# hammershock/3dgs-avatar-release

Measured on AMD Instinct MI355X. Metric: render fps (fwd+bwd) @200k Gaussians 1024x1024 SH3, higher is better.
Workload: dtype f32; 1 GPU; config3: 200k Gaussians, 1024x1024, SH deg 3, forward+backward; shs+scales+rotations inputs, L1 loss (L1 fused into the rasterizer: l1_target); tile_rect=1, l1=fused, long_lists=0, gaussians=200000, width=1024, height=1024, sh_degree=3, frames_per_rank=1857, total_frames=1857, ranks=1, backend=none, parallelism=frames sharded x1

## Files before the change

### 3dgs-avatar-release_amd/csrc/render_bwd.hip

```cpp
#include "common.h"
#include "blend.h"

__device__ __forceinline__ float ring_ror1(float v) {
    return __builtin_bit_cast(float, __builtin_amdgcn_update_dpp(0, __builtin_bit_cast(int, v), 0x121, 0xF, 0xF, true));
}
#define RING 16
#define RING_STRIDE 48

typedef float bwd_f4 __attribute__((ext_vector_type(4)));
template <bool SECOND>
__device__ __forceinline__ void split_accumulate(float (&x)[9], float (&y)[9], unsigned long long mask, float Gd, float dx,
                                                 float dy, float tdx, float tdy, float wgt, float gx, float gy,
                                                 float gz, unsigned long long m1, uint32_t lds_addr, bwd_f4& q0, bwd_f4& q1,
                                                 bwd_f4& q2, float& rot0, float& rot1) {
    unsigned long long save;
    asm volatile(
        "s_mov_b64 %[sv], exec\n\t"
        "s_mov_b64 exec, %[m]\n\t"
        "v_fmac_f32 %[x0], %[Gd], %[dx]\n\t"
        "v_fmac_f32 %[x1], %[Gd], %[dy]\n\t"
        "v_fmac_f32 %[x2], %[tdx], %[dx]\n\t"
        "v_fmac_f32 %[x3], %[tdx], %[dy]\n\t"
        "v_fmac_f32 %[x4], %[tdy], %[dy]\n\t"
        "v_add_f32 %[x5], %[x5], %[Gd]\n\t"
        "v_fmac_f32 %[x6], %[w], %[gx]\n\t"
        "v_fmac_f32 %[x7], %[w], %[gy]\n\t"
        "v_fmac_f32 %[x8], %[w], %[gz]\n\t"
        "s_mov_b64 exec, %[sv]"
        : [x0] "+v"(x[0]), [x1] "+v"(x[1]), [x2] "+v"(x[2]), [x3] "+v"(x[3]), [x4] "+v"(x[4]), [x5] "+v"(x[5]), [x6] "+v"(x[6]),
          [x7] "+v"(x[7]), [x8] "+v"(x[8]), [sv] "=&s"(save)
        : [m] "s"(mask), [Gd] "v"(Gd), [dx] "v"(dx), [dy] "v"(dy), [tdx] "v"(tdx), [tdy] "v"(tdy), [w] "v"(wgt), [gx] "v"(gx),
          [gy] "v"(gy), [gz] "v"(gz)
        : "scc");
#define GS_ACC_Y                                     \
        "s_andn2_b64 exec, %[sv], %[m]\n\t"          \
        "v_fmac_f32 %[y0], %[Gd], %[dx]\n\t"         \
        "v_fmac_f32 %[y1], %[Gd], %[dy]\n\t"         \
        "v_fmac_f32 %[y2], %[tdx], %[dx]\n\t"        \
        "v_fmac_f32 %[y3], %[tdx], %[dy]\n\t"        \
        "v_fmac_f32 %[y4], %[tdy], %[dy]\n\t"        \
        "v_add_f32 %[y5], %[y5], %[Gd]\n\t"          \
        "v_fmac_f32 %[y6], %[w], %[gx]\n\t"          \
        "v_fmac_f32 %[y7], %[w], %[gy]\n\t"          \
        "v_fmac_f32 %[y8], %[w], %[gz]\n\t"          \
        "s_mov_b64 exec, %[sv]\n\t"                  \
        "v_mov_b32_dpp %[r0], %[r0] row_ror:1 row_mask:0xf bank_mask:0xf bound_ctrl:1\n\t" \
        "v_mov_b32_dpp %[r1], %[r1] row_ror:1 row_mask:0xf bank_mask:0xf bound_ctrl:1\n\t" \
        "s_waitcnt lgkmcnt(0)"
#define GS_ACC_Y_OUT [y0] "+v"(y[0]), [y1] "+v"(y[1]), [y2] "+v"(y[2]), [y3] "+v"(y[3]), [y4] "+v"(y[4]), [y5] "+v"(y[5]), \
                     [y6] "+v"(y[6]), [y7] "+v"(y[7]), [y8] "+v"(y[8]), [q0] "+v"(q0), [q1] "+v"(q1), [r0] "+v"(rot0), [r1] "+v"(rot1), \
                     [sv] "=&s"(save)
#define GS_ACC_Y_IN [m] "s"(mask), [m1] "s"(m1), [a] "v"(lds_addr), [Gd] "v"(Gd), [dx] "v"(dx), [dy] "v"(dy), [tdx] "v"(tdx), \
                    [tdy] "v"(tdy), [w] "v"(wgt), [gx] "v"(gx), [gy] "v"(gy), [gz] "v"(gz)
    if constexpr (SECOND) {
        asm volatile(
            "s_mov_b64 %[sv], exec\n\t"
            "s_andn2_b64 exec, %[m1], %[m]\n\t"
            "ds_read_b128 %[q0], %[a]\n\t"
            "ds_read_b128 %[q1], %[a] offset:16\n\t"
            "ds_read_b128 %[q2], %[a] offset:32\n\t" GS_ACC_Y
            : GS_ACC_Y_OUT, [q2] "+v"(q2)
            : GS_ACC_Y_IN
            : "memory", "scc");
    } else {
        asm volatile(
            "s_mov_b64 %[sv], exec\n\t"
            "s_andn2_b64 exec, %[m1], %[m]\n\t"
            "ds_read_b128 %[q0], %[a]\n\t"
            "ds_read_b128 %[q1], %[a] offset:16\n\t"
            "ds_read_b32 %[q2], %[a] offset:32\n\t" GS_ACC_Y
            : GS_ACC_Y_OUT, [q2] "+v"(q2.x)
            : GS_ACC_Y_IN
            : "memory", "scc");
    }
#undef GS_ACC_Y
#undef GS_ACC_Y_OUT
#undef GS_ACC_Y_IN
}

struct EntryQ {
    bwd_f4 q0, q1, q2;
};
#define ENT_SLOTS 2

template <bool SECOND>
__device__ __forceinline__ void switch_entry(EntryQ& e, uint32_t lds_addr, unsigned long long m0, unsigned long long m1) {
    unsigned long long save;
    if constexpr (SECOND) {
        asm volatile(
            "s_mov_b64 %[sv], exec\n\t"
            "s_andn2_b64 exec, %[m1], %[m0]\n\t"
            "ds_read_b128 %[q0], %[a]\n\t"
            "ds_read_b128 %[q1], %[a] offset:16\n\t"
            "ds_read_b128 %[q2], %[a] offset:32\n\t"
            "s_mov_b64 exec, %[sv]\n\t"
            "s_waitcnt lgkmcnt(0)"
            : [q0] "+v"(e.q0), [q1] "+v"(e.q1), [q2] "+v"(e.q2), [sv] "=&s"(save)
            : [a] "v"(lds_addr), [m0] "s"(m0), [m1] "s"(m1)
            : "memory", "scc");
    } else {
        float b = e.q2.x;
        asm volatile(
            "s_mov_b64 %[sv], exec\n\t"
            "s_andn2_b64 exec, %[m1], %[m0]\n\t"
            "ds_read_b128 %[q0], %[a]\n\t"
            "ds_read_b128 %[q1], %[a] offset:16\n\t"
            "ds_read_b32 %[b], %[a] offset:32\n\t"
            "s_mov_b64 exec, %[sv]\n\t"
            "s_waitcnt lgkmcnt(0)"
            : [q0] "+v"(e.q0), [q1] "+v"(e.q1), [b] "+v"(b), [sv] "=&s"(save)
            : [a] "v"(lds_addr), [m0] "s"(m0), [m1] "s"(m1)
            : "memory", "scc");
        e.q2.x = b;
    }
}

#ifndef BWD_MIN_WAVES
#define BWD_MIN_WAVES 1
#endif
template <int MODE>
__global__ __launch_bounds__(64, BWD_MIN_WAVES) void render_bwd_kernel(const float4* __restrict__ rec,
                                                        const uint2* __restrict__ ranges,
                                                        const uint32_t* __restrict__ order, int W, int H, int gx,
                                                        int ntiles, int xmap,
                                                        const uint32_t* __restrict__ qlist,
                                                        const uint32_t* __restrict__ ncon_c,
                                                        const uint32_t* __restrict__ qcount,
                                                        const float* __restrict__ out_color,
                                                        const float* __restrict__ dL_dpix,
                                                        const float* __restrict__ dL_dopa,
                                                        const float* __restrict__ final_T, const float* __restrict__ bg,
                                                        float4* __restrict__ qrows, uint32_t* __restrict__ q8,
                                                        const float4* __restrict__ ckpt,
                                                        const uint32_t* __restrict__ ck_start, const int chunks,
                                                        const int blocks_per_chunk, const SecondImage second,
                                                        const L1Grad l1, const float l1_inv_n) {
    constexpr bool OPA = MODE == 1, SECOND = MODE == 2, SONES = MODE == 3;
    if constexpr (SECOND) { if (*second.all_ones != 0u) return; }
    if constexpr (SONES) { if (*second.all_ones == 0u) return; }
    constexpr int NP2 = SECOND ? 5 : 3;
    __shared__ float2 pix[NP2][4 * RING_STRIDE];
    __shared__ bwd_f4 ent[ENT_SLOTS][RING][3];
    int slot, q;
    const int chunk = chunks > 1 ? (int)blockIdx.x / blocks_per_chunk : 0;
    render_block_map((int)blockIdx.x - chunk * blocks_per_chunk, xmap, &slot, &q);
    if (slot >= ntiles) return;
    const int tile = (int)(order[slot] & 0x7FFFFFFFu);
    const int tx = tile % gx, ty = tile / gx;
    const int lane = threadIdx.x;
    const int j = lane & (RING - 1), ring = lane / RING;
    const int QX0 = tx * TILE + 8 * (q & 1), QY0 = ty * TILE + 8 * (q >> 1);
    const int px = QX0 + (lane & 7), py = QY0 + (lane >> 3);
    const uint2 range = ranges[tile];
    const int n = (int)(range.y - range.x);
    const int m_all = (int)qcount[tile * 4 + q];
    const uint32_t ks = chunk > 0 ? ck_start[(size_t)(tile * 4 + q) * (size_t)chunks + chunk] : 0u;
    if (ks >= (uint32_t)m_all) return;
    const int k0 = (int)ks;
    const uint32_t ke = chunk + 1 < chunks ? ck_start[(size_t)(tile * 4 + q) * (size_t)chunks + chunk + 1] : 0xFFFFFFFFu;
    const int m = (int)min(ke, (uint32_t)m_all) - k0;
    const uint32_t qbase = 4u * range.x + (uint32_t)q * (uint32_t)n + (uint32_t)k0;
    const float4 zero4 = make_float4(0.f, 0.f, 0.f, 0.f);
    float gtot0, T0 = 1.0f;
    {
        float4 c0 = zero4, c1 = make_float4((float)px, (float)py, __uint_as_float((uint32_t)j), 0.f);
        float3 h = make_float3(0.f, 0.f, 0.f);
        if (px < W && py < H) {
            const size_t HW = (size_t)H * W;
            const size_t pid = (size_t)py * W + px;
            float g0 = 0.f, g1 = 0.f, g2 = 0.f;
            if (dL_dpix) { g0 = dL_dpix[pid]; g1 = dL_dpix[HW + pid]; g2 = dL_dpix[2 * HW + pid]; }
            const float o0 = out_color[pid], o1 = out_color[HW + pid], o2 = out_color[2 * HW + pid];
            if (l1.target) {
                const float sc = (l1.grad ? l1.grad[0] : 1.0f) * l1_inv_n;
                const float d0 = o0 - l1.target[pid], d1 = o1 - l1.target[HW + pid], d2 = o2 - l1.target[2 * HW + pid];
                g0 += d0 > 0.f ? sc : (d0 < 0.f ? -sc : 0.f);
                g1 += d1 > 0.f ? sc : (d1 < 0.f ? -sc : 0.f);
                g2 += d2 > 0.f ? sc : (d2 < 0.f ? -sc : 0.f);
            }
            c0 = make_float4(g0, g1, g2, o0 * g0 + o1 * g1 + o2 * g2);
            const uint32_t nc = ncon_c[pid];
            c1.z = __uint_as_float((nc > (uint32_t)k0 ? nc - (uint32_t)k0 : 0u) + (uint32_t)j);
            if (OPA) {
                const float Tf = final_T[pid];
                c0.w -= dL_dopa[pid] * (Tf * (1.0f - bg[0]));
            }
            if (SECOND || SONES) {
                h = make_float3(second.dL_dpix[pid], second.dL_dpix[HW + pid], second.dL_dpix[2 * HW + pid]);
                if (SECOND) c0.w += second.out_color[pid] * h.x + second.out_color[HW + pid] * h.y + second.out_color[2 * HW + pid] * h.z;
                else c0.w -= (1.0f - second.out_color[pid]) * h.x + (1.0f - second.out_color[HW + pid]) * h.y + (1.0f - second.out_color[2 * HW + pid]) * h.z;
            }
            if (chunk > 0) {
                const size_t ci = ((size_t)(tile * 4 + q) * (size_t)(chunks - 1) + (size_t)(chunk - 1)) * 64 + lane;
                const float4 ck = ckpt[ci];
                T0 = ck.x;
                c0.w -= ck.y * g0 + ck.z * g1 + ck.w * g2;
                if (SECOND) {
                    const float4 ck2 = second.ckpt[ci];
                    c0.w -= ck2.y * h.x + ck2.z * h.y + ck2.w * h.z;
                }
            }
        }
        const int slot = ring * RING_STRIDE + j;
        pix[0][slot] = pix[0][slot + RING] = make_float2(c0.x, c0.y);
        pix[1][slot] = pix[1][slot + RING] = make_float2(c0.z, c1.x);
        pix[2][slot] = pix[2][slot + RING] = make_float2(c1.y, c1.z);
        if (SECOND) {
            pix[3][slot] = pix[3][slot + RING] = make_float2(h.x, h.y);
            pix[4][slot] = pix[4][slot + RING] = make_float2(h.z, 0.f);
        }
        gtot0 = c0.w;
    }

    float3 q2 = make_float3(0.f, 0.f, 0.f);
    auto stage = [&](const float4 p0, const float4 p1, const float4 p2, const int chunk, uint32_t& row) {
        const uint32_t off = __float_as_uint(p2.y), rmin = __float_as_uint(p2.z), rsz = __float_as_uint(p2.w);
        const uint32_t minx = rmin & 0xFFFFu, miny = rmin >> 16, w = rsz & 0xFFFFu;
        row = gradient_row(off, w, (uint32_t)tx - minx, (uint32_t)ty - miny, (uint32_t)q);
        if (ring == 0) {
            bwd_f4* e = ent[chunk & (ENT_SLOTS - 1)][j];
            e[0] = bwd_f4{p0.x, p0.y, (-0.5f * LOG2E_F) * p0.z, -LOG2E_F * p0.w};
            e[1] = bwd_f4{(-0.5f * LOG2E_F) * p1.x, p1.y, p1.z, p1.w};
            e[2] = bwd_f4{p2.x, q2.x, q2.y, q2.z};
        }
    };
    auto gather = [&](int k, float4& p0, float4& p1, float4& p2) {
        if (k < m) {
            const uint32_t id = qlist[qbase + k];
            p0 = rec[(size_t)id * 3];
            p1 = rec[(size_t)id * 3 + 1];
            p2 = rec[(size_t)id * 3 + 2];
            if (SECOND) q2 = make_float3(second.colors[(size_t)id * 3], second.colors[(size_t)id * 3 + 1], second.colors[(size_t)id * 3 + 2]);
        }
    };

    float4 p0 = zero4, p1 = zero4, p2 = zero4;
    EntryQ cur;
    cur.q0 = cur.q1 = cur.q2 = bwd_f4{0.f, 0.f, 0.f, 0.f};
    uint32_t row_staged = 0;
    gather(j, p0, p1, p2);
    stage(p0, p1, p2, 0, row_staged);
    gather(RING + j, p0, p1, p2);
    __syncthreads();
    const uint32_t ent_addr0 = (uint32_t)(uintptr_t)&ent[0][j][0], ent_addr1 = (uint32_t)(uintptr_t)&ent[1][j][0];

    float accA[9], accB[9];
#pragma unroll
    for (int c9 = 0; c9 < 9; c9++) accA[c9] = accB[c9] = 0.f;
    uint32_t rowA = 0, rowB = 0;
    uint32_t pidx = (uint32_t)(ring * RING_STRIDE + ((RING - j) & (RING - 1)));
    float2 pc[NP2];
#pragma unroll
    for (int c6 = 0; c6 < NP2; c6++) pc[c6] = pix[c6][pidx];
    float T = __shfl(T0, ring * RING + ((RING - j) & (RING - 1)), 64);
    float Rem = __shfl(gtot0, ring * RING + ((RING - j) & (RING - 1)), 64);

    auto write_row = [&](size_t row, const float* a) {
        qrows[row * 2] = make_float4(a[0], a[1], a[2], a[3]);
        qrows[row * 2 + 1] = make_float4(a[4], a[5], a[6], a[7]);
        q8[row] = __float_as_uint(a[8]);
    };

    const int total = m + RING - 1;
    auto fold_rings = [&](float (&a)[9]) {
#pragma unroll
        for (int c9 = 0; c9 < 9; c9++) {
            a[c9] += __shfl_xor(a[c9], 16, 64);
            a[c9] += __shfl_xor(a[c9], 32, 64);
        }
    };
    auto run_round = [&](const int s0, float (&X)[9], uint32_t& rowX, float (&Y)[9]) {
        if (s0 >= 2 * RING) {
            fold_rings(X);
            if (ring == 0) write_row(rowX, X);
        }
        rowX = row_staged;
        const uint32_t ea = (s0 & RING) ? ent_addr1 : ent_addr0;
        switch_entry<SECOND>(cur, ea, 0ull, 0x0001000100010001ull);
        stage(p0, p1, p2, s0 / RING + 1, row_staged);
        gather(s0 + 2 * RING + j, p0, p1, p2);
        if (s0 > 0) pidx -= (uint32_t)RING;
#pragma unroll
        for (int c9 = 0; c9 < 9; c9++) X[c9] = 0.f;
        const int tend = min(RING, total - s0);
        unsigned long long mx = 0x0001000100010001ull;
        auto step = [&](const int t) {
            const uint32_t s = (uint32_t)(s0 + t);
            const float3 g = make_float3(pc[0].x, pc[0].y, pc[1].x);
            const float pxf = pc[1].y, pyf = pc[2].x;
            const uint32_t lim = __float_as_uint(pc[2].y);
            const float h0 = SECOND ? pc[3].x : 0.f, h1 = SECOND ? pc[3].y : 0.f, h2 = SECOND ? pc[NP2 - 1].x : 0.f;
            pidx += 1u;
#pragma unroll
            for (int c6 = 0; c6 < NP2; c6++) pc[c6] = pix[c6][pidx];
            const float dx = cur.q0.x - pxf, dy = cur.q0.y - pyf;
            const float power2 = __builtin_fmaf(cur.q0.z * dx, dx, __builtin_fmaf(cur.q0.w, dx, cur.q1.x * dy) * dy);
            const float G = __builtin_amdgcn_exp2f(power2);
            const float al = fminf(0.99f, cur.q1.y * G);
            const bool valid = (power2 <= 0.0f) && (s < lim) && (al >= (1.0f / 255.0f));
            const float alpha = valid ? al : 0.f;
            const float Gv = valid ? G : 0.f;
            const float wgt = alpha * T;
            float cg = cur.q1.z * g.x + cur.q1.w * g.y + cur.q2.x * g.z;
            if constexpr (SECOND) cg += cur.q2.y * h0 + cur.q2.z * h1 + cur.q2.w * h2;
            Rem = __builtin_fmaf(-cg, wgt, Rem);
            const float one_m = 1.f - alpha;
            const float dL_dalpha = T * cg - Rem * __builtin_amdgcn_rcpf(one_m);
            T *= one_m;
            const float Gd = Gv * dL_dalpha;
            const float tdx = Gd * dx, tdy = Gd * dy;
            const unsigned long long mx1 = (mx << 1) | 0x0001000100010001ull;
            split_accumulate<SECOND>(X, Y, mx, Gd, dx, dy, tdx, tdy, wgt, g.x, g.y, g.z, mx1, ea, cur.q0, cur.q1, cur.q2, T, Rem);
            mx = mx1;
        };
        int t = 0;
        for (; t + 1 < tend; t += 2) {
            step(t);
            step(t + 1);
        }
        if (t < tend) step(t);
    };
    for (int s0 = 0; s0 < total; s0 += 2 * RING) {
        run_round(s0, accA, rowA, accB);
        if (s0 + RING < total) run_round(s0 + RING, accB, rowB, accA);
    }
    {
        const int last_round = (total - 1) / RING;
        const bool odd = last_round & 1;
        const int k_new = RING * last_round + j, k_old = k_new - RING;
        fold_rings(accA);
        fold_rings(accB);
        if (ring == 0) {
            if (k_new <= m - 1) write_row(odd ? rowB : rowA, odd ? accB : accA);
            if (last_round >= 1 && k_old <= m - 1) write_row(odd ? rowA : rowB, odd ? accA : accB);
        }
    }
}

int launch_render_backward(const float* rec, const uint32_t* ranges, const uint32_t* order, int W, int H,
                           const QuadLists& ql, const float* out_color, const float* dL_dpix, const float* dL_dopa,
                           const float* final_T, const float* bg, float* qrows, uint32_t* q8, const SecondImage* second,
                           L1Grad l1, hipStream_t s) {
    const int gx = (W + TILE - 1) / TILE, gy = (H + TILE - 1) / TILE;
    const int xmap = gs_tune_get(GS_TUNE_XCD_MAP);
    const int chunks = ql.ckpt ? ql.chunks : 1;
    const int bpc = render_grid_blocks(gx * gy, xmap);
    const dim3 grid((unsigned)bpc * (unsigned)chunks);
    const SecondImage none{nullptr, nullptr, nullptr, nullptr, nullptr};
    const float l1_inv_n = 1.0f / (3.0f * (float)W * (float)H);
#define GS_BWD_ARGS                                                                                                       \
    reinterpret_cast<const float4*>(rec), reinterpret_cast<const uint2*>(ranges), order, W, H, gx, gx * gy, xmap, ql.qlist, \
        ql.ncon_c, ql.qcount, out_color, dL_dpix, dL_dopa, final_T, bg, reinterpret_cast<float4*>(qrows), q8, ql.ckpt,    \
        ql.ck_start, chunks, bpc
    if (second) {
        hipLaunchKernelGGL(render_bwd_kernel<2>, grid, dim3(64), 0, s, GS_BWD_ARGS, *second, l1, l1_inv_n);
        hipLaunchKernelGGL(render_bwd_kernel<3>, grid, dim3(64), 0, s, GS_BWD_ARGS, *second, l1, l1_inv_n);
    } else if (dL_dopa)
        hipLaunchKernelGGL(render_bwd_kernel<1>, grid, dim3(64), 0, s, GS_BWD_ARGS, none, l1, l1_inv_n);
    else
        hipLaunchKernelGGL(render_bwd_kernel<0>, grid, dim3(64), 0, s, GS_BWD_ARGS, none, l1, l1_inv_n);
#undef GS_BWD_ARGS
    GS_LAUNCH_CHECK("render_backward", 0, s);
    return GS_OK;
}
```

Before: 1761 frames/s.

## Pipeline id prefetch, permlane-swap ring folding, and pre-rotated pixel layout in bwd

Pixels are now assigned to lanes in the pre-rotated order, so the initial T/Rem shuffles are no longer needed. The qlist id load is issued one round earlier than the record gather so the two loads overlap instead of forming a dependent chain. The ring reduction now uses v_permlane16/32_swap instead of shfl_xor, and all four rings each write part of the output row rather than only ring 0. The kernel also caps waves per EU at 6 and returns early when a chunk is empty; the lower occupancy cap and the gfx950-specific permlane asm add register-pressure and portability risk.

```diff
diff --git a/3dgs-avatar-release_amd/csrc/render_bwd.hip b/3dgs-avatar-release_amd/csrc/render_bwd.hip
--- a/3dgs-avatar-release_amd/csrc/render_bwd.hip
+++ b/3dgs-avatar-release_amd/csrc/render_bwd.hip
@@ -118,7 +118,11 @@
 #ifndef BWD_MIN_WAVES
 #define BWD_MIN_WAVES 1
 #endif
+#ifndef BWD_MAX_WAVES
+#define BWD_MAX_WAVES (BWD_MIN_WAVES > 6 ? BWD_MIN_WAVES : 6)
+#endif
 template <int MODE>
+__attribute__((amdgpu_waves_per_eu(BWD_MIN_WAVES, BWD_MAX_WAVES)))
 __global__ __launch_bounds__(64, BWD_MIN_WAVES) void render_bwd_kernel(const float4* __restrict__ rec,
                                                         const uint2* __restrict__ ranges,
                                                         const uint32_t* __restrict__ order, int W, int H, int gx,
@@ -150,7 +154,8 @@
     const int lane = threadIdx.x;
     const int j = lane & (RING - 1), ring = lane / RING;
     const int QX0 = tx * TILE + 8 * (q & 1), QY0 = ty * TILE + 8 * (q >> 1);
-    const int px = QX0 + (lane & 7), py = QY0 + (lane >> 3);
+    const int pi = (RING - j) & (RING - 1), pl = ring * RING + pi;
+    const int px = QX0 + (pl & 7), py = QY0 + (pl >> 3);
     const uint2 range = ranges[tile];
     const int n = (int)(range.y - range.x);
     const int m_all = (int)qcount[tile * 4 + q];
@@ -159,11 +164,12 @@
     const int k0 = (int)ks;
     const uint32_t ke = chunk + 1 < chunks ? ck_start[(size_t)(tile * 4 + q) * (size_t)chunks + chunk + 1] : 0xFFFFFFFFu;
     const int m = (int)min(ke, (uint32_t)m_all) - k0;
+    if (m <= 0) return;
     const uint32_t qbase = 4u * range.x + (uint32_t)q * (uint32_t)n + (uint32_t)k0;
     const float4 zero4 = make_float4(0.f, 0.f, 0.f, 0.f);
     float gtot0, T0 = 1.0f;
     {
-        float4 c0 = zero4, c1 = make_float4((float)px, (float)py, __uint_as_float((uint32_t)j), 0.f);
+        float4 c0 = zero4, c1 = make_float4((float)px, (float)py, __uint_as_float((uint32_t)pi), 0.f);
         float3 h = make_float3(0.f, 0.f, 0.f);
         if (px < W && py < H) {
             const size_t HW = (size_t)H * W;
@@ -180,7 +186,7 @@
             }
             c0 = make_float4(g0, g1, g2, o0 * g0 + o1 * g1 + o2 * g2);
             const uint32_t nc = ncon_c[pid];
-            c1.z = __uint_as_float((nc > (uint32_t)k0 ? nc - (uint32_t)k0 : 0u) + (uint32_t)j);
+            c1.z = __uint_as_float((nc > (uint32_t)k0 ? nc - (uint32_t)k0 : 0u) + (uint32_t)pi);
             if (OPA) {
                 const float Tf = final_T[pid];
                 c0.w -= dL_dopa[pid] * (Tf * (1.0f - bg[0]));
@@ -191,7 +197,7 @@
                 else c0.w -= (1.0f - second.out_color[pid]) * h.x + (1.0f - second.out_color[HW + pid]) * h.y + (1.0f - second.out_color[2 * HW + pid]) * h.z;
             }
             if (chunk > 0) {
-                const size_t ci = ((size_t)(tile * 4 + q) * (size_t)(chunks - 1) + (size_t)(chunk - 1)) * 64 + lane;
+                const size_t ci = ((size_t)(tile * 4 + q) * (size_t)(chunks - 1) + (size_t)(chunk - 1)) * 64 + pl;
                 const float4 ck = ckpt[ci];
                 T0 = ck.x;
                 c0.w -= ck.y * g0 + ck.z * g1 + ck.w * g2;
@@ -201,7 +207,7 @@
                 }
             }
         }
-        const int slot = ring * RING_STRIDE + j;
+        const int slot = ring * RING_STRIDE + pi;
         pix[0][slot] = pix[0][slot + RING] = make_float2(c0.x, c0.y);
         pix[1][slot] = pix[1][slot + RING] = make_float2(c0.z, c1.x);
         pix[2][slot] = pix[2][slot + RING] = make_float2(c1.y, c1.z);
@@ -224,23 +230,26 @@
             e[2] = bwd_f4{p2.x, q2.x, q2.y, q2.z};
         }
     };
-    auto gather = [&](int k, float4& p0, float4& p1, float4& p2) {
-        if (k < m) {
-            const uint32_t id = qlist[qbase + k];
-            p0 = rec[(size_t)id * 3];
-            p1 = rec[(size_t)id * 3 + 1];
-            p2 = rec[(size_t)id * 3 + 2];
-            if (SECOND) q2 = make_float3(second.colors[(size_t)id * 3], second.colors[(size_t)id * 3 + 1], second.colors[(size_t)id * 3 + 2]);
-        }
+    uint32_t id_ahead = 0;
+    auto gather_id = [&](int k) { id_ahead = qlist[qbase + min(k, m - 1)]; };
+    auto gather = [&](float4& p0, float4& p1, float4& p2) {
+        const uint32_t id = id_ahead;
+        p0 = rec[(size_t)id * 3];
+        p1 = rec[(size_t)id * 3 + 1];
+        p2 = rec[(size_t)id * 3 + 2];
+        if (SECOND) q2 = make_float3(second.colors[(size_t)id * 3], second.colors[(size_t)id * 3 + 1], second.colors[(size_t)id * 3 + 2]);
     };
 
     float4 p0 = zero4, p1 = zero4, p2 = zero4;
     EntryQ cur;
     cur.q0 = cur.q1 = cur.q2 = bwd_f4{0.f, 0.f, 0.f, 0.f};
     uint32_t row_staged = 0;
-    gather(j, p0, p1, p2);
+    gather_id(j);
+    gather(p0, p1, p2);
+    gather_id(RING + j);
     stage(p0, p1, p2, 0, row_staged);
-    gather(RING + j, p0, p1, p2);
+    gather(p0, p1, p2);
+    gather_id(2 * RING + j);
     __syncthreads();
     const uint32_t ent_addr0 = (uint32_t)(uintptr_t)&ent[0][j][0], ent_addr1 = (uint32_t)(uintptr_t)&ent[1][j][0];
 
@@ -248,37 +257,62 @@
 #pragma unroll
     for (int c9 = 0; c9 < 9; c9++) accA[c9] = accB[c9] = 0.f;
     uint32_t rowA = 0, rowB = 0;
-    uint32_t pidx = (uint32_t)(ring * RING_STRIDE + ((RING - j) & (RING - 1)));
+    uint32_t pidx = (uint32_t)(ring * RING_STRIDE + pi);
     float2 pc[NP2];
 #pragma unroll
     for (int c6 = 0; c6 < NP2; c6++) pc[c6] = pix[c6][pidx];
-    float T = __shfl(T0, ring * RING + ((RING - j) & (RING - 1)), 64);
-    float Rem = __shfl(gtot0, ring * RING + ((RING - j) & (RING - 1)), 64);
-
-    auto write_row = [&](size_t row, const float* a) {
-        qrows[row * 2] = make_float4(a[0], a[1], a[2], a[3]);
-        qrows[row * 2 + 1] = make_float4(a[4], a[5], a[6], a[7]);
-        q8[row] = __float_as_uint(a[8]);
+    float T = T0, Rem = gtot0;
+
+    auto fold_rings = [&](float (&a)[9], float (&f)[3]) {
+        float t;
+        asm volatile(
+            "s_nop 1\n\t"
+            "v_permlane16_swap_b32 %[a0], %[a1]\n\t"
+            "v_permlane16_swap_b32 %[a2], %[a3]\n\t"
+            "v_permlane16_swap_b32 %[a4], %[a5]\n\t"
+            "v_permlane16_swap_b32 %[a6], %[a7]\n\t"
+            "v_mov_b32 %[t], %[a8]\n\t"
+            "v_add_f32 %[a0], %[a0], %[a1]\n\t"
+            "v_add_f32 %[a2], %[a2], %[a3]\n\t"
+            "v_add_f32 %[a4], %[a4], %[a5]\n\t"
+            "v_add_f32 %[a6], %[a6], %[a7]\n\t"
+            "v_permlane16_swap_b32 %[a8], %[t]\n\t"
+            "v_permlane32_swap_b32 %[a0], %[a2]\n\t"
+            "v_permlane32_swap_b32 %[a4], %[a6]\n\t"
+            "v_add_f32 %[a8], %[a8], %[t]\n\t"
+            "v_add_f32 %[a0], %[a0], %[a2]\n\t"
+            "v_add_f32 %[a4], %[a4], %[a6]\n\t"
+            "v_mov_b32 %[t], %[a8]\n\t"
+            "s_nop 1\n\t"
+            "v_permlane32_swap_b32 %[a8], %[t]\n\t"
+            "v_add_f32 %[a8], %[a8], %[t]"
+            : [a0] "+v"(a[0]), [a1] "+v"(a[1]), [a2] "+v"(a[2]), [a3] "+v"(a[3]), [a4] "+v"(a[4]), [a5] "+v"(a[5]),
+              [a6] "+v"(a[6]), [a7] "+v"(a[7]), [a8] "+v"(a[8]), [t] "=&v"(t));
+        f[0] = a[0];
+        f[1] = a[4];
+        f[2] = a[8];
+    };
+    float* const qrow_words = reinterpret_cast<float*>(qrows);
+    auto write_row = [&](size_t row, const float (&f)[3]) {
+        qrow_words[row * 8 + ring] = f[0];
+        qrow_words[row * 8 + ring + 4] = f[1];
+        if (ring == 0) q8[row] = __float_as_uint(f[2]);
     };
 
     const int total = m + RING - 1;
-    auto fold_rings = [&](float (&a)[9]) {
-#pragma unroll
-        for (int c9 = 0; c9 < 9; c9++) {
-            a[c9] += __shfl_xor(a[c9], 16, 64);
-            a[c9] += __shfl_xor(a[c9], 32, 64);
-        }
-    };
     auto run_round = [&](const int s0, float (&X)[9], uint32_t& rowX, float (&Y)[9]) {
-        if (s0 >= 2 * RING) {
-            fold_rings(X);
-            if (ring == 0) write_row(rowX, X);
-        }
+        const uint32_t row_done = rowX;
         rowX = row_staged;
         const uint32_t ea = (s0 & RING) ? ent_addr1 : ent_addr0;
         switch_entry<SECOND>(cur, ea, 0ull, 0x0001000100010001ull);
         stage(p0, p1, p2, s0 / RING + 1, row_staged);
-        gather(s0 + 2 * RING + j, p0, p1, p2);
+        gather(p0, p1, p2);
+        gather_id(s0 + 3 * RING + j);
+        if (s0 >= 2 * RING) {
+            float f[3];
+            fold_rings(X, f);
+            write_row(row_done, f);
+        }
         if (s0 > 0) pidx -= (uint32_t)RING;
 #pragma unroll
         for (int c9 = 0; c9 < 9; c9++) X[c9] = 0.f;
@@ -328,12 +362,11 @@
         const int last_round = (total - 1) / RING;
         const bool odd = last_round & 1;
         const int k_new = RING * last_round + j, k_old = k_new - RING;
-        fold_rings(accA);
-        fold_rings(accB);
-        if (ring == 0) {
-            if (k_new <= m - 1) write_row(odd ? rowB : rowA, odd ? accB : accA);
-            if (last_round >= 1 && k_old <= m - 1) write_row(odd ? rowA : rowB, odd ? accA : accB);
-        }
+        float fA[3], fB[3];
+        fold_rings(accA, fA);
+        fold_rings(accB, fB);
+        if (k_new <= m - 1) write_row(odd ? rowB : rowA, odd ? fB : fA);
+        if (last_round >= 1 && k_old <= m - 1) write_row(odd ? rowA : rowB, odd ? fA : fB);
     }
 }
 
```

After: 1803 frames/s (median of 6 runs). 2.3% higher.
